# Totoketchup/Adaptive-MultiSpeaker-Separation

Measured on AMD Instinct MI355X. Metric: mixtures/sec training throughput (2-spk, 256-filter adapt+BLSTM-DPCL), higher is better.
Workload: dtype f32 (storage, accumulation and results f32; dense products issued on the 16-bit matrix pipe as fp16x3 / bf16x6 emulation of the f32 product -- `value_native_f32` is the same step on v_mfma_f32_32x32x2_f32)

## Files before the change

adaptive-multispeaker-separation_amd/csrc/common.h:

```cpp
#pragma once
#include <hip/hip_runtime.h>
#include <stdint.h>
#include <stddef.h>
#include "../../include/ams.h"

typedef float f32x4 __attribute__((ext_vector_type(4)));
typedef float f32x16 __attribute__((ext_vector_type(16)));

extern thread_local int g_ams_last_hip_error;

static inline ams_status ams_check_launch() {
    hipError_t e = hipGetLastError();
    if (e != hipSuccess) {
        g_ams_last_hip_error = (int)e;
        return AMS_E_LAUNCH_FAILED;
    }
    return AMS_OK;
}

#define AMS_REQUIRE(cond)            \
    do {                             \
        if (!(cond)) return AMS_E_INVALID_ARG; \
    } while (0)

static inline int ceil_div(long a, long b) { return (int)((a + b - 1) / b); }

namespace ams_detail {
size_t conv_maxpool_ps_bytes(int Bt, int L, int W, int N);
bool conv_maxpool_ps_applies(int Bt, int L, int W, int N);
ams_status conv_maxpool_ps(const float* x, const float* f, float* pmax, int32_t* pidx, int Bt, int L, int W, int N, int pl,
                           const float* amax_x, const float* amax_f, void* img, hipStream_t st);
int dx_splits(int M, int N, int K, size_t ws_bytes, int* kps);
ams_status splitk_reduce(const float* partial, float* C, int M, int N, long ldc, int splits, hipStream_t st);
ams_status conv_fwd_or_dx(const float* x, const float* w, const float* bias, float* y, int M, int N, int T, int F, int lc, int kh, int kw,
                          int rt, int rf, int relu, const float* emask, const float* amax_a, const float* amax_b, float* amax_out,
                          hipStream_t st);
ams_status conv_wgrad(const float* x, const float* dy, float* dw, float* db, float* bsum_ws, int P, int N, int T, int F, int lc, int kh,
                      int kw, int rt, int rf, const float* amax_a, const float* amax_b, void* ws, size_t ws_bytes, hipStream_t st);
size_t conv_wgrad_ws_bytes(int P, int N, int Mrows);
}

__device__ __forceinline__ float wave_sum(float v) {
#pragma unroll
    for (int o = 32; o > 0; o >>= 1) v += __shfl_xor(v, o, 64);
    return v;
}
template <int S>
__device__ __forceinline__ float lane_above(float v) {
    const unsigned b = __builtin_bit_cast(unsigned, v);
    if constexpr (S == 32 || S == 16) {
        unsigned hi = b, lo = 0u;
        if constexpr (S == 32) asm volatile("s_nop 1\n\tv_permlane32_swap_b32 %0, %1\n\ts_nop 1" : "+v"(hi), "+v"(lo));
        else asm volatile("s_nop 1\n\tv_permlane16_swap_b32 %0, %1\n\ts_nop 1" : "+v"(hi), "+v"(lo));
        return __builtin_bit_cast(float, lo);
    }
    else return __builtin_bit_cast(float, __builtin_amdgcn_update_dpp(0u, b, 0x100 | S, 0xf, 0xf, true));
}

__device__ __forceinline__ float wave_sum_lane0(float v) {
    v += lane_above<32>(v);
    v += lane_above<16>(v);
    v += lane_above<8>(v);
    v += lane_above<4>(v);
    v += lane_above<2>(v);
    v += lane_above<1>(v);
// ... 14 lines not shown
```

adaptive-multispeaker-separation_amd/csrc/gemm.hip:

```cpp
#include "common.h"
#include "split.h"
#include <stdlib.h>
#include <atomic>
#include <type_traits>

namespace {

struct LaunchOpt { const float* amax_a = nullptr; const float* amax_b = nullptr; int lds_pad = 0; void* sk_scratch = nullptr; size_t sk_bytes = 0;
                   unsigned* amax_out = nullptr; int force_cfg = -1; };
constexpr size_t AMS_SK_FLAG_BYTES = 8192;
constexpr size_t AMS_SK_SLOT_BYTES = (128 * 256 + 256) * sizeof(float);
std::atomic<int> g_gemm_arith{-1};

struct GemmTuning { int group_m, splits, x6cfg, sk; bool novec, f16x3; };
inline const GemmTuning& tuning() {
    static const GemmTuning t = [] {
        GemmTuning v{0, 0, -1, 1, false, true};
        if (const char* f = getenv("AMS_GEMM_SK")) v.sk = atoi(f);
        if (const char* f = getenv("AMS_GEMM_GROUP_M")) v.group_m = atoi(f);
        if (const char* f = getenv("AMS_GEMM_SPLITS")) v.splits = atoi(f);
        { const char* e = getenv("AMS_GEMM_F16X3"); v.f16x3 = !(e && atoi(e) == 0); }
        v.novec = getenv("AMS_GEMM_NOVEC") != nullptr;
        if (const char* f = getenv("AMS_GEMM_X6CFG")) { const int c = atoi(f); if (c == 0 || c == 3) v.x6cfg = c; }
        return v;
    }();
    return t;
}

#ifndef AMS_GEMM_BK
#define AMS_GEMM_BK 8
#endif
inline bool use_x6() {
    int v = g_gemm_arith.load(std::memory_order_relaxed);
    if (v < 0) {
        const char* f = getenv("AMS_GEMM_X6");
        v = (f && atoi(f) == 0) ? 0 : 1;
        g_gemm_arith.store(v, std::memory_order_relaxed);
    }
    return v != 0;
}
constexpr int BM = 128, BN = 128, BK = AMS_GEMM_BK;
constexpr int X6_BK = 32;
#ifndef AMS_GEMM_X6_US16
#define AMS_GEMM_X6_US16 0.84
#endif
#ifndef AMS_X6_OCC1
#define AMS_X6_OCC1 1
#endif
#ifndef AMS_GEMM_X6_US16_2
#define AMS_GEMM_X6_US16_2 1.35
#endif
constexpr int PAD_T = 2;
constexpr int PAD_V = 4;

enum { A_ROW = 0, A_COL = 1, A_FRAMES = 2, A_FRAMES_T = 3, A_CONV = 4, A_CONV_T = 5 };
// ... 1295 lines not shown
    p.grid = (unsigned)G;
    p.t = wgcu * ((R * nkf + sk_kt) * tk + (R + 1) * 5.0 + 3.0 + 2.0 * contrib) / occ;
    return p;
}

template <int AMODE, int BMODE>
ams_status launch(GemmArgs& g, const LaunchOpt& opt, void* ws, size_t ws_bytes, hipStream_t st, int nbatch = 1,
                  float* bsum_out = nullptr, int bsum_accumulate = 0, float* bsum_ws = nullptr) {
    constexpr bool AKc = (AMODE == A_ROW || AMODE == A_CONV), BKcc = (BMODE == B_COL);
    const int lds_pad = opt.lds_pad < 0 ? 0 : opt.lds_pad;
    const bool capped = lds_pad > 0;
    const bool vec_off = tuning().novec;
    const bool vec = g.a_vec && g.b_vec && !vec_off &&
                     (AMODE == A_FRAMES ? (g.K % 4 == 0 && g.fr_L >= 4) : AMODE == A_FRAMES_T ? (g.M % 4 == 0 && g.fr_L >= 4) :
                      AKc ? (g.K % 4 == 0 && g.K >= 4) : (g.M % 4 == 0 && g.M >= 4)) &&
                     (BKcc ? (g.K % 4 == 0 && g.K >= 4) : (g.N % 4 == 0 && g.N >= 4));
    const bool x6 = vec && use_x6();
    const int cfg = x6 ? ((opt.force_cfg == 0 || opt.force_cfg == 3) && tuning().x6cfg < 0 ? opt.force_cfg : x6_choose_cfg(g.M, g.N)) : 0;
    const bool f16 = x6 && opt.amax_a && opt.amax_b && tuning().f16x3;
    g.amax_a = f16 ? opt.amax_a : nullptr;
    g.amax_b = f16 ? opt.amax_b : nullptr;
    g.amax_out = x6 ? opt.amax_out : nullptr;
    g.c_vec = (g.N % 4 == 0) && (g.ldc % 4 == 0) && (g.c_zs % 4 == 0) && (g.bias_zs % 4 == 0) &&
              (((uintptr_t)g.C | (uintptr_t)ws | (uintptr_t)g.bias) & 15) == 0;
    if (opt.amax_out && !x6) return AMS_E_INVALID_ARG;
    const TilePlan tp = x6 ? x6_plan(cfg) : f32_plan();
    const int tiles = ceil_div(g.M, tp.bm) * ceil_div(g.N, tp.bn);
    g.group_m = choose_group_m(ceil_div(g.M, tp.bm), ceil_div(g.N, tp.bn));
    int splits = 1;
    double t_split = 1e30;
    const bool whole = opt.amax_out || g.relu || g.emask;
    if (ws && !whole) {
        splits = choose_splits(g.M, g.N, g.K, nbatch, tp, &t_split);
        if (tuning().splits > 0) splits = tuning().splits;
        while (splits > 1 && (size_t)nbatch * splits * g.M * g.N * sizeof(float) > ws_bytes) --splits;
    } else choose_splits(g.M, g.N, g.K, nbatch, tp, &t_split, 1);
    int wgcu = 1;
    if (x6 && cfg == 0) { wgcu = capped ? 163840 / (17152 + lds_pad) : 2; if (wgcu < 1) wgcu = 1; if (wgcu > 2) wgcu = 2; }
    SkPlan sk;
    g.sk_rounds = -1; g.sk_flags = nullptr; g.sk_slots = nullptr; g.sk_slot_floats = 0; g.amax_fold = 0;
    if (x6 && !capped && opt.sk_scratch && tuning().sk != 0 && tuning().splits <= 0) {
        sk = sk_plan(tiles * nbatch, g.K, tp, wgcu);
        const size_t slot = (size_t)(tp.bm * tp.bn + tp.bn) * sizeof(float);
        if (sk.rounds >= 0 && (opt.sk_bytes < AMS_SK_FLAG_BYTES + (size_t)sk.grid * slot || (((uintptr_t)opt.sk_scratch) & 15))) sk.rounds = -1;
        if (sk.rounds >= 0 && tuning().sk == 1 && !(sk.t < 0.97 * t_split)) sk.rounds = -1;
        if (sk.rounds == 0 && tuning().sk == 1 && !opt.amax_out) sk.rounds = -1;
        if (sk.rounds >= 0) {
            splits = 1;
            g.sk_rounds = sk.rounds;
            g.sk_flags = (int*)opt.sk_scratch;
            g.sk_slots = (float*)((char*)opt.sk_scratch + AMS_SK_FLAG_BYTES);
            g.sk_slot_floats = (int)(slot / sizeof(float));
        }
    }
    int kps = ceil_div(g.K, splits);
    kps = ceil_div(kps, tp.bk) * tp.bk;
    splits = ceil_div(g.K, kps);
    if (whole && splits > 1) return AMS_E_INVALID_ARG;
    g.splits = splits;
    g.k_per_split = kps;
    g.partial = (float*)ws;
    g.bsum_part = bsum_out ? bsum_ws : nullptr;
    const bool bsum_in_launch = x6 && bsum_out && splits == 1 && (((uintptr_t)bsum_out) & 15) == 0;
    if (sk.rounds >= 0 && bsum_out && !bsum_in_launch) return AMS_E_INVALID_ARG;
    g.bsum_out = bsum_in_launch ? bsum_out : nullptr;
    g.bsum_accumulate = bsum_accumulate;
    g.nbatch = nbatch;
    dim3 grid((unsigned)((long)tiles * splits * nbatch));
// ... 42 lines not shown
    ams_status s = ams_check_launch();
    if (s != AMS_OK) return s;
    if (splits > 1) {
        const long total = (long)g.M * g.N;
        const bool rvec = (g.N % 4 == 0) && (g.ldc % 4 == 0) && (g.c_zs % 4 == 0) && (g.bias_zs % 4 == 0) &&
                          (((uintptr_t)g.C | (uintptr_t)g.partial | (uintptr_t)g.bias) & 15) == 0 && total < (1L << 31);
        if (rvec) {
            int blocks = (int)((total / 4 + 255) / 256);
            if (blocks > 4096) blocks = 4096;
            hipLaunchKernelGGL(splitk_reduce_vec_kernel, dim3(blocks, nbatch), dim3(256), 0, st, g.partial, g.C, g.bias, g.M, g.N, g.ldc,
                               splits, g.accumulate, g.c_zs, g.bias_zs);
        } else {
            int blocks = (int)((total + 255) / 256);
            if (blocks > 2048) blocks = 2048;
            hipLaunchKernelGGL(splitk_reduce_kernel, dim3(blocks, nbatch), dim3(256), 0, st, g.partial, g.C, g.bias, g.M, g.N, g.ldc,
                               splits, g.accumulate, g.c_zs, g.bias_zs);
        }
        s = ams_check_launch();
    }
    if (s == AMS_OK && bsum_out && !bsum_in_launch) {
        if (!vec || BMODE != B_ROW) return AMS_E_INVALID_ARG;
        hipLaunchKernelGGL(bsum_finish_kernel, dim3(ceil_div(g.N, 256)), dim3(256), 0, st, bsum_ws, bsum_out, g.N, splits, bsum_accumulate);
        s = ams_check_launch();
    }
    return s;
}

inline bool aligned16(const void* p) { return ((uintptr_t)p & 15) == 0; }

}

namespace ams_detail {

__attribute__((visibility("hidden"))) int dx_splits(int M, int N, int K, size_t ws_bytes, int* kps) {
    int splits = choose_splits(M, N, K, 1, x6_plan(3));
    if (tuning().splits > 0) splits = tuning().splits;
    while (splits > 1 && (size_t)splits * M * N * sizeof(float) > ws_bytes) --splits;
    int k = ceil_div(ceil_div(K, splits), X6_BK) * X6_BK;
    *kps = k;
    return ceil_div(K, k);
}

__attribute__((visibility("hidden"))) ams_status splitk_reduce(const float* partial, float* C, int M, int N, long ldc, int splits, hipStream_t st) {
    const long total = (long)M * N;
    if (N % 4 || ldc % 4 || (((uintptr_t)C | (uintptr_t)partial) & 15) || total >= (1L << 31)) return AMS_E_INVALID_ARG;
    int blocks = (int)((total / 4 + 255) / 256);
    if (blocks > 4096) blocks = 4096;
    hipLaunchKernelGGL(splitk_reduce_vec_kernel, dim3(blocks, 1), dim3(256), 0, st, partial, C, (const float*)nullptr, M, N, ldc, splits, 0, 0L, 0L);
    return ams_check_launch();
}


__attribute__((visibility("hidden"))) ams_status conv_fwd_or_dx(const float* x, const float* w, const float* bias, float* y, int M, int N,
                                                              int T, int F, int lc, int kh, int kw, int rt, int rf, int relu,
                                                              const float* emask, const float* amax_a, const float* amax_b, float* amax_out,
                                                              hipStream_t st) {
    GemmArgs g{};
    g.A = x; g.B = w; g.C = y; g.bias = bias;
    g.M = M; g.N = N; g.K = kh * kw * (1 << lc); g.lda = 0; g.ldb = N; g.ldc = N;
    g.cv_T = T; g.cv_F = F; g.cv_lc = lc; g.cv_kh = kh; g.cv_kw = kw; g.cv_rt = rt; g.cv_rf = rf;
    g.relu = relu; g.emask = emask;
    g.a_vec = aligned16(x) && lc >= 2;
    g.b_vec = aligned16(w) && (N % 4 == 0);
    LaunchOpt o; o.amax_a = amax_a; o.amax_b = amax_b;
    const bool x6 = use_x6() && g.a_vec && g.b_vec && !tuning().novec && g.K >= 4 && N >= 4;
    if (amax_out && x6) o.amax_out = reinterpret_cast<unsigned*>(amax_out);
    ams_status s = launch<A_CONV, B_ROW>(g, o, nullptr, 0, st);
    if (s == AMS_OK && amax_out && !x6) s = ams_absmax_f32(y, (long)M * N, amax_out, st);
    return s;
}
__attribute__((visibility("hidden"))) ams_status conv_wgrad(const float* x, const float* dy, float* dw, float* db, float* bsum_ws, int P, int N,
                                                          int T, int F, int lc, int kh, int kw, int rt, int rf, const float* amax_a,
                                                          const float* amax_b, void* ws, size_t ws_bytes, hipStream_t st) {
    GemmArgs g{};
    g.A = x; g.B = dy; g.C = dw; g.bias = nullptr;
    g.M = kh * kw * (1 << lc); g.N = N; g.K = P; g.lda = 0; g.ldb = N; g.ldc = N;
    g.cv_T = T; g.cv_F = F; g.cv_lc = lc; g.cv_kh = kh; g.cv_kw = kw; g.cv_rt = rt; g.cv_rf = rf;
    g.a_vec = aligned16(x) && lc >= 2;
    g.b_vec = aligned16(dy) && (N % 4 == 0);
    LaunchOpt o; o.amax_a = amax_a; o.amax_b = amax_b;
    return launch<A_CONV_T, B_ROW>(g, o, ws, ws_bytes, st, 1, db, 0, bsum_ws);
}
size_t conv_wgrad_ws_bytes(int P, int N, int Mrows) { return ams_gemm_workspace_bytes(Mrows, N, P, 1, 0); }

}

extern "C" {

void ams_gemm_set_arith(int mode) { g_gemm_arith.store(mode ? 1 : 0, std::memory_order_relaxed); }
int ams_gemm_get_arith(void) { return use_x6() ? 1 : 0; }

size_t ams_gemm_sk_scratch_bytes(void) {
    const size_t g8 = (size_t)(device_cus() + 7) / 8 * 8;
    const size_t a = g8 * 2 * (128 * 128 + 128) * sizeof(float), b = g8 * AMS_SK_SLOT_BYTES;
    return AMS_SK_FLAG_BYTES + (a > b ? a : b);
}

size_t ams_gemm_workspace_bytes(int M, int N, int K, int nbatch, int lds_pad) {
    if (M <= 0 || N <= 0 || K <= 0 || nbatch <= 0) return 0;
    int splits = choose_splits(M, N, K, nbatch);
    if (tuning().splits > 0) splits = tuning().splits;
    return slab_bytes(M, N, nbatch, splits);
}

ams_status ams_gemm_f32_at_b_colsum(int M, int N, int K, const float* A, long lda, const float* B, long ldb, float* C, long ldc,
                                    int accumulate, float* bsum_out, int bsum_accumulate, float* bsum_ws, const float* amax_a,
                                    const float* amax_b, int lds_pad, void* ws, size_t ws_bytes, void* sk_scratch, size_t sk_bytes,
                                    void* stream) {
    AMS_REQUIRE(M > 0 && N > 0 && K > 0 && A && B && C && bsum_out && bsum_ws);
    GemmArgs g{};
    g.A = A; g.B = B; g.C = C;
    g.M = M; g.N = N; g.K = K; g.lda = lda; g.ldb = ldb; g.ldc = ldc;
    g.accumulate = accumulate;
    g.a_vec = aligned16(A) && (lda % 4 == 0);
    g.b_vec = aligned16(B) && (ldb % 4 == 0);
    AMS_REQUIRE(g.a_vec && g.b_vec && M % 4 == 0 && N % 4 == 0 && aligned16(bsum_ws) && !tuning().novec);
    LaunchOpt o; o.amax_a = amax_a; o.amax_b = amax_b; o.lds_pad = lds_pad; o.sk_scratch = sk_scratch; o.sk_bytes = sk_bytes;
    return launch<A_COL, B_ROW>(g, o, ws, ws_bytes, (hipStream_t)stream, 1, bsum_out, bsum_accumulate, bsum_ws);
}

struct BwGroupPlan { int M[3], N[3], K[3], splits[3], kps[3], tiles_m[3], tiles_n[3]; size_t slab_off[3], bsum_off, bytes; int n_items; };
static bool bw_group_plan(int B, int T, int D, int H, BwGroupPlan& p) {
    if (B <= 0 || T <= 0 || D <= 0 || H <= 0 || D % 4 || H % 4 || (long)B * T < 2 || (long)B * T >= (1L << 31) / (8L * H) ||
        (long)(D + H) * 8 * H >= (1L << 31)) return false;
    const TilePlan tp = x6_plan(3);
    const int Kall = B * T;
    const int M[3] = {D, H, H}, N[3] = {8 * H, 4 * H, 4 * H}, K[3] = {Kall, Kall - 1, Kall - 1};
    int tiles = 0;
    double elems = 0.0;
    for (int r = 0; r < 3; ++r) {
        p.M[r] = M[r]; p.N[r] = N[r]; p.K[r] = K[r];
        p.tiles_m[r] = ceil_div(M[r], tp.bm); p.tiles_n[r] = ceil_div(N[r], tp.bn);
        tiles += p.tiles_m[r] * p.tiles_n[r];
        elems += (double)M[r] * N[r];
// ... 655 lines not shown
```

adaptive-multispeaker-separation_amd/csrc/gemm_ps.hip:

```cpp
#include "common.h"
#include "split.h"
#include <type_traits>

namespace {

typedef __attribute__((address_space(3))) void lds_void;

constexpr int PS_BK = 32, PS_BM = 128, PS_BN = 256, PS_NT = 512;
constexpr int PS_A_BYTES = PS_BM * 128, PS_B_BYTES = PS_BN * 128, PS_STAGE = PS_A_BYTES + PS_B_BYTES;
constexpr int PS_STAGES = 3;
constexpr int PS_BIAS_OFF = PS_STAGES * PS_STAGE;
constexpr int PS_LDS = PS_BIAS_OFF + 2 * 1024;


__device__ __forceinline__ void ps_pack_rows_body(const float* __restrict__ x, long ldx, unsigned char* __restrict__ img,
                                                  unsigned pitch, int R, int K, const float* __restrict__ amax, unsigned block) {
    const int groups = (int)(pitch / 32);
    const long id = (long)block * 256 + threadIdx.x;
    if (id >= (long)R * groups) return;
    const int r = (int)(id / groups), gq = (int)(id - (long)r * groups), k = gq * 8;
    const float s = f16_scale(amax[0]);
    float v[8];
    const float* row = x + (long)r * ldx;
    if (k + 8 <= K && ((((uintptr_t)(row + k)) & 15) == 0)) {
// ... 433 lines not shown
        const bool cok = col < g.N;
        const float4 bv = AF32 ? float4{0.f, 0.f, 0.f, 0.f} : *reinterpret_cast<const float4*>(ps_smem + PS_BIAS_OFF + (wi & 1) * 1024 + (wn * 64 + c4) * 4);
        float* const out = (AF32 && g.splits > 1) ? g.partial + (long)split * g.M * g.N : g.C;
        const long ldo = (AF32 && g.splits > 1) ? (long)g.N : g.ldc;
#pragma unroll
        for (int i = 0; i < 2; ++i) {
#pragma unroll
            for (int j = 0; j < 2; ++j) {
                acc[i][j] = (acc[i][j] + accs[i][j]) * sc_inv;
#pragma unroll
                for (int r = 0; r < 16; ++r) wl[((r & 3) + 8 * (r >> 2) + 4 * lk) * 64 + j * 32 + l31] = acc[i][j][r];
            }
#pragma unroll
            for (int p8 = 0; p8 < 8; ++p8) {
                const int rl = p8 * 4 + rr;
                float4 v = *reinterpret_cast<const float4*>(wl + rl * 64 + c4);
                const int row = em0 + (wm * 2 + i) * 32 + rl;
                if (row < g.M && cok) {
                    if constexpr (!AF32) { v.x += bv.x; v.y += bv.y; v.z += bv.z; v.w += bv.w; }
                    *reinterpret_cast<float4*>(out + (long)row * ldo + col) = v;
                }
            }
        }
        PS_STAMP(2);
        if (more) {
            asm volatile("s_waitcnt lgkmcnt(0)" ::: "memory");
            __builtin_amdgcn_s_barrier();
            if constexpr (AF32) { setup(wi + 1); start_af32(); }
            else if (nk > 1) issue(1, 1);
        }
    }
}

inline int ps_group_m(int tiles_m, int tiles_n) {
    int gm = 8;
    if (gm > tiles_m) gm = tiles_m;
    (void)tiles_n;
    return gm < 1 ? 1 : gm;
}

}

extern "C" {

size_t ams_ps_image_pitch(int K) { return (size_t)((K + 31) / 32) * 128; }
size_t ams_ps_image_bytes(int rows, int K) { return (size_t)rows * ams_ps_image_pitch(K); }

ams_status ams_ps_pack_rows(const float* x, long ldx, void* img, int R, int K, const float* amax, void* stream) {
    AMS_REQUIRE(x && img && amax && R > 0 && K > 0 && ldx >= K && (((uintptr_t)img) & 15) == 0);
    const unsigned pitch = (unsigned)ams_ps_image_pitch(K);
    const long n = (long)R * (pitch / 32);
    hipLaunchKernelGGL(ps_pack_rows_kernel, dim3((unsigned)((n + 255) / 256)), dim3(256), 0, (hipStream_t)stream, x, ldx, (unsigned char*)img, pitch, R, K, amax);
    return ams_check_launch();
}

ams_status ams_ps_pack_cols(const float* w, long ldw, void* img, int K, int N, const float* amax, void* stream) {
    AMS_REQUIRE(w && img && amax && K > 0 && N > 0 && ldw >= N && (((uintptr_t)img) & 15) == 0);
    const unsigned pitch = (unsigned)ams_ps_image_pitch(K);
    hipLaunchKernelGGL(ps_pack_cols_kernel, dim3((unsigned)((N + 63) / 64), (unsigned)(((K + 31) / 32 + PS_PC_KT - 1) / PS_PC_KT)), dim3(256), 0, (hipStream_t)stream, w, ldw,
                       (unsigned char*)img, pitch, K, N, amax);
    return ams_check_launch();
}

ams_status ams_ps_pack_many(const ams_ps_pack_region* regions, int n, int max_workgroups, int lds_pad, void* stream) {
    AMS_REQUIRE(regions && n >= 1 && n <= AMS_PS_PACK_MAX && max_workgroups >= 0 && lds_pad >= 0 && lds_pad <= 150 * 1024);
    PsPackTable tab{};
// ... 12 lines not shown
        tab.r[i] = g;
    }
    tab.blocks = (unsigned)blocks;
    static const bool raised = [] { return hipFuncSetAttribute((const void*)ps_pack_many_kernel, hipFuncAttributeMaxDynamicSharedMemorySize, 150 * 1024) == hipSuccess; }();
    if (!raised) return AMS_E_LAUNCH_FAILED;
    const unsigned grid = (max_workgroups > 0 && (unsigned long)max_workgroups < blocks) ? (unsigned)max_workgroups : (unsigned)blocks;
    hipLaunchKernelGGL(ps_pack_many_kernel, dim3(grid), dim3(256), (size_t)lds_pad, (hipStream_t)stream, tab);
    return ams_check_launch();
}

ams_status ams_gemm_ps(int M, int N, int K, const void* A_img, const void* B_img, float* C, long ldc, const float* bias, const float* amax_a,
                       const float* amax_b, void* stream) {
    AMS_REQUIRE(A_img && B_img && C && amax_a && amax_b && M > 0 && N > 0 && K > 0);
    AMS_REQUIRE(N % 4 == 0 && ldc % 4 == 0 && ldc >= N && ((((uintptr_t)C) | ((uintptr_t)bias) | ((uintptr_t)A_img) | ((uintptr_t)B_img)) & 15) == 0);
    PsArgs g{};
    g.A = (const unsigned char*)A_img; g.B = (const unsigned char*)B_img; g.C = C; g.bias = bias; g.amax_a = amax_a; g.amax_b = amax_b;
    g.M = M; g.N = N; g.K = K; g.ldc = ldc;
    g.pitch_a = g.pitch_b = (unsigned)ams_ps_image_pitch(K);
    AMS_REQUIRE((long)M * g.pitch_a < (1L << 31) && (long)N * g.pitch_b < (1L << 31));
    g.tiles_m = (M + PS_BM - 1) / PS_BM; g.tiles_n = (N + PS_BN - 1) / PS_BN;
    g.group_m = ps_group_m(g.tiles_m, g.tiles_n);
    static const int cus = [] { int dev = 0, n = 0; if (hipGetDevice(&dev) != hipSuccess || hipDeviceGetAttribute(&n, hipDeviceAttributeMultiprocessorCount, dev) != hipSuccess || n <= 0) n = 256; return n; }();
    static const bool raised = [] { return hipFuncSetAttribute((const void*)gemm_ps_kernel<false>, hipFuncAttributeMaxDynamicSharedMemorySize, PS_LDS) == hipSuccess; }();
    if (!raised) return AMS_E_LAUNCH_FAILED;
    const int items = g.tiles_m * g.tiles_n;
    int grid = items < cus ? items : cus;
    if (grid >= 8) grid -= grid % 8;
    hipLaunchKernelGGL(gemm_ps_kernel<false>, dim3((unsigned)grid), dim3(PS_NT), PS_LDS, (hipStream_t)stream, g);
    return ams_check_launch();
}

size_t ams_gemm_ps_a_workspace_bytes(int M, int N, int K) {
    if (M <= 0 || N <= 0 || K <= 0) return 0;
    int kps = 0;
    const int splits = ams_detail::dx_splits(M, N, K, ~(size_t)0, &kps);
    return splits > 1 ? (size_t)splits * M * N * sizeof(float) : 0;
}

ams_status ams_gemm_ps_a_f32(int M, int N, int K, const float* A, long lda, const void* B_img, float* C, long ldc, const float* amax_a,
                             const float* amax_b, void* ws, size_t ws_bytes, void* stream) {
    AMS_REQUIRE(A && B_img && C && amax_a && amax_b && M > 0 && N > 0 && K > 0 && lda >= K);
    AMS_REQUIRE(N % 4 == 0 && ldc % 4 == 0 && ldc >= N && lda % 4 == 0 &&
                ((((uintptr_t)C) | ((uintptr_t)A) | ((uintptr_t)B_img) | ((uintptr_t)ws)) & 15) == 0);
    PsArgs g{};
    g.Af = A; g.lda = lda; g.B = (const unsigned char*)B_img; g.C = C; g.bias = nullptr; g.amax_a = amax_a; g.amax_b = amax_b;
    g.M = M; g.N = N; g.K = K; g.ldc = ldc;
    g.pitch_b = (unsigned)ams_ps_image_pitch(K);
    AMS_REQUIRE((long)M * lda * 4 < (1L << 31) && (long)N * g.pitch_b < (1L << 31));
    g.splits = ams_detail::dx_splits(M, N, K, ws ? ws_bytes : 0, &g.kps);
    g.partial = (float*)ws;
    g.tiles_m = (M + PS_BM - 1) / PS_BM; g.tiles_n = (N + PS_BN - 1) / PS_BN;
    g.group_m = ps_group_m(g.tiles_m, g.tiles_n);
    static const int cus = [] { int dev = 0, n = 0; if (hipGetDevice(&dev) != hipSuccess || hipDeviceGetAttribute(&n, hipDeviceAttributeMultiprocessorCount, dev) != hipSuccess || n <= 0) n = 256; return n; }();
    static const bool raised = [] { return hipFuncSetAttribute((const void*)gemm_ps_kernel<false, true>, hipFuncAttributeMaxDynamicSharedMemorySize, PS_LDS) == hipSuccess; }();
    if (!raised) return AMS_E_LAUNCH_FAILED;
    const int items = g.tiles_m * g.tiles_n * g.splits;
    int grid = items < cus ? items : cus;
    if (grid >= 8) grid -= grid % 8;
    hipLaunchKernelGGL((gemm_ps_kernel<false, true>), dim3((unsigned)grid), dim3(PS_NT), PS_LDS, (hipStream_t)stream, g);
    ams_status r = ams_check_launch();
    if (r == AMS_OK && g.splits > 1) r = ams_detail::splitk_reduce(g.partial, C, M, N, ldc, g.splits, (hipStream_t)stream);
    return r;
}

}

namespace ams_detail {

static inline unsigned conv_lpp(int L, int W) { return (unsigned)((L - 1) / 8 + 4 * ((W + 31) / 32) + 1); }

__attribute__((visibility("hidden"))) size_t conv_maxpool_ps_bytes(int Bt, int L, int W, int N) {
    const size_t a = (size_t)8 * 2 * Bt * conv_lpp(L, W) * 16, b = ams_ps_image_bytes(N, W);
    return (a + 255) / 256 * 256 + (b + 255) / 256 * 256;
}
__attribute__((visibility("hidden"))) bool conv_maxpool_ps_applies(int Bt, int L, int W, int N) {
    return L % PS_BM == 0 && N % 4 == 0 && (size_t)8 * 2 * Bt * conv_lpp(L, W) * 16 < ((size_t)1 << 31) - 64 && ams_ps_image_bytes(N, W) < ((size_t)1 << 31);
}

__attribute__((visibility("hidden"))) ams_status conv_maxpool_ps(const float* x, const float* f, float* pmax, int32_t* pidx, int Bt, int L, int W,
                                                                 int N, int pl, const float* amax_x, const float* amax_f, void* img,
                                                                 hipStream_t st) {
    const unsigned lpp = conv_lpp(L, W);
    const size_t a_bytes = (size_t)8 * 2 * Bt * lpp * 16;
    unsigned char* const ia = (unsigned char*)img;
    unsigned char* const ib = ia + (a_bytes + 255) / 256 * 256;
    const long pieces = (long)8 * Bt * lpp;
    hipLaunchKernelGGL(ps_pack_conv_kernel, dim3((unsigned)((pieces + 255) / 256)), dim3(256), 0, st, x, ia, Bt, L, pl, lpp, amax_x);
    ams_status r = ams_ps_pack_cols(f, N, ib, W, N, amax_f, st);
    if (r != AMS_OK) return r;
    PsArgs g{};
    g.A = ia; g.B = ib; g.C = pmax; g.pidx = pidx; g.bias = nullptr; g.amax_a = amax_x; g.amax_b = amax_f;
    g.M = Bt * L; g.N = N; g.K = W; g.ldc = N;
// ... 16 lines not shown
```

include/ams.h:

```cpp
#ifndef AMS_H
#define AMS_H
#include <stddef.h>
#include <stdint.h>

#ifdef __cplusplus
extern "C" {
#endif

#define AMS_ABI_VERSION 10

typedef int32_t ams_status;
#define AMS_OK 0
#define AMS_E_INVALID_ARG (-1)
#define AMS_E_WORKSPACE_TOO_SMALL (-2)
#define AMS_E_LAUNCH_FAILED (-3)

int ams_last_error(void);
int ams_abi_version(void);

ams_status ams_front_filter_fwd(const float* w, const float* bases, float* f, int W, int N, void* stream);
ams_status ams_front_filter_bwd(const float* w, const float* bases, const float* df, float* dw, float* dbases, int W, int N,
                                void* stream);

size_t ams_front_conv_fwd_workspace_bytes(int Bt, int L, int W, int N, int hop);
// ... 18 lines not shown
                                int P, int hop, int S, void* stream);
ams_status ams_synth_unpool_bwd_vals(const float* dout, const int32_t* pos, const float* f2t, float* dvals, int R, int L, int W, int N,
                                     int T, int S, void* stream);

size_t ams_gemm_workspace_bytes(int M, int N, int K, int nbatch, int lds_pad);
size_t ams_gemm_sk_scratch_bytes(void);
void ams_gemm_set_arith(int mode);
int ams_gemm_get_arith(void);
ams_status ams_gemm_f32(int transA, int transB, int M, int N, int K, const float* A, long lda, const float* B, long ldb, float* C,
                        long ldc, const float* bias, int accumulate, int mask_period, int mask_skip, const float* amax_a,
                        const float* amax_b, int lds_pad, void* ws, size_t ws_bytes, void* sk_scratch, size_t sk_bytes, void* stream);
size_t ams_ps_image_pitch(int K);
size_t ams_ps_image_bytes(int rows, int K);
ams_status ams_ps_pack_rows(const float* x, long ldx, void* img, int R, int K, const float* amax, void* stream);
ams_status ams_ps_pack_cols(const float* w, long ldw, void* img, int K, int N, const float* amax, void* stream);
#define AMS_PS_PACK_MAX 8
#define AMS_PS_PACK_ROWS 0
#define AMS_PS_PACK_COLS 1
typedef struct ams_ps_pack_region {
    const float* src;
    long ld;
    void* img;
    const float* amax;
    int K;
    int rows;
    int kind;
    unsigned pitch;
    unsigned first_block;
} ams_ps_pack_region;
ams_status ams_ps_pack_many(const ams_ps_pack_region* regions, int n, int max_workgroups, int lds_pad, void* stream);
ams_status ams_gemm_ps(int M, int N, int K, const void* A_img, const void* B_img, float* C, long ldc, const float* bias,
                       const float* amax_a, const float* amax_b, void* stream);
size_t ams_gemm_ps_a_workspace_bytes(int M, int N, int K);
ams_status ams_gemm_ps_a_f32(int M, int N, int K, const float* A, long lda, const void* B_img, float* C, long ldc, const float* amax_a,
                             const float* amax_b, void* ws, size_t ws_bytes, void* stream);

ams_status ams_gemm_f32_at_b_colsum(int M, int N, int K, const float* A, long lda, const float* B, long ldb, float* C, long ldc,
                                    int accumulate, float* bsum_out, int bsum_accumulate, float* bsum_ws, const float* amax_a,
                                    const float* amax_b, int lds_pad, void* ws, size_t ws_bytes, void* sk_scratch, size_t sk_bytes,
                                    void* stream);
size_t ams_blstm_bwd_weights_workspace_bytes(int B, int T, int D, int H, int lds_pad);
ams_status ams_blstm_bwd_weights_f32(int B, int T, int D, int H, const float* x, long ldx, const float* h, const float* dz, float* dK,
                                     long ldk, float* db, int accumulate, const float* bound_x, const float* bound_h, const float* bound_dz,
                                     int lds_pad, void* ws, size_t ws_bytes, void* stream);
size_t ams_dilated_conv2d_workspace_bytes(int B, int T, int F, int cin, int cout, int kh, int kw);
ams_status ams_dilated_conv2d_fwd(const float* x, const float* w, const float* bias, float* y, int B, int T, int F, int cin, int cout,
                                  int kh, int kw, int rt, int rf, const float* amax_x, const float* amax_w, float* amax_y, void* ws,
                                  size_t ws_bytes, void* stream);
ams_status ams_dilated_conv2d_bwd_data(const float* dy, const float* w, const float* y_below, float* dx, int B, int T, int F, int cin,
                                       int cout, int kh, int kw, int rt, int rf, const float* amax_dy, const float* amax_w,
                                       float* amax_dx, void* ws, size_t ws_bytes, void* stream);
ams_status ams_dilated_conv2d_bwd_filter(const float* x, const float* dy, float* dw, float* db, int B, int T, int F, int cin,
                                         int cout, int kh, int kw, int rt, int rf, const float* amax_x, const float* amax_dy, void* ws,
                                         size_t ws_bytes, void* stream);
ams_status ams_dilated_conv2d_relu_bwd(const float* dy, const float* y, float* dx, long n, float* amax_dx, void* stream);
ams_status ams_gemm_f32_batched(int transA, int transB, int M, int N, int K, const float* A, long lda, long a_zs, const float* B,
                                long ldb, long b_zs, float* C, long ldc, long c_zs, int nbatch, int accumulate, int mask_period,
                                int mask_skip, const float* amax_a, const float* amax_b, int lds_pad, void* ws, size_t ws_bytes,
                                void* sk_scratch, size_t sk_bytes, void* stream);
ams_status ams_range_share(const float* x, long rows, long cols, long ld, const float* bound, float* out3, void* stream);
ams_status ams_absmax_f32(const float* x, long n, float* out, void* stream);

ams_status ams_make_masks(const float* rep_non_mix, float* Y, int32_t* argmax, int B, int S, long TF, float a, float b,
                          int take_abs, void* stream);

size_t ams_blstm_pack_floats(int H, int backward);
// ... 156 lines not shown
```

Baseline: 24500.

## Add 128x320 wide-tile f16x3 dx GEMM kernel chosen by a cost model

Adds a new pre-split f16x3 GEMM kernel with a 320-column tile: five MFMA blocks per wave, a three-stage B pipeline and direct-to-LDS buffer loads. A planner (dx_plan) compares modeled time for the 256 and 320 tiles and picks the tile and split-K count, and the generic GEMM path and workspace sizing now use it. The aim is more reuse of each A tile and fewer tiles or partial slabs for wide-N data-gradient GEMMs. The cost is higher LDS and register use, one workgroup per CU, and a 320 estimate that is just the 256 per-tile cost scaled by 1.25.

```diff
diff --git a/adaptive-multispeaker-separation_amd/csrc/common.h b/adaptive-multispeaker-separation_amd/csrc/common.h
--- a/adaptive-multispeaker-separation_amd/csrc/common.h
+++ b/adaptive-multispeaker-separation_amd/csrc/common.h
@@ -30,7 +30,8 @@
 bool conv_maxpool_ps_applies(int Bt, int L, int W, int N);
 ams_status conv_maxpool_ps(const float* x, const float* f, float* pmax, int32_t* pidx, int Bt, int L, int W, int N, int pl,
                            const float* amax_x, const float* amax_f, void* img, hipStream_t st);
-int dx_splits(int M, int N, int K, size_t ws_bytes, int* kps);
+struct DxPlan { int tile_n, splits, kps; };
+DxPlan dx_plan(int M, int N, int K, size_t ws_bytes);
 ams_status splitk_reduce(const float* partial, float* C, int M, int N, long ldc, int splits, hipStream_t st);
 ams_status conv_fwd_or_dx(const float* x, const float* w, const float* bias, float* y, int M, int N, int T, int F, int lc, int kh, int kw,
                           int rt, int rf, int relu, const float* emask, const float* amax_a, const float* amax_b, float* amax_out,
diff --git a/adaptive-multispeaker-separation_amd/csrc/gemm.hip b/adaptive-multispeaker-separation_amd/csrc/gemm.hip
--- a/adaptive-multispeaker-separation_amd/csrc/gemm.hip
+++ b/adaptive-multispeaker-separation_amd/csrc/gemm.hip
@@ -12,15 +12,16 @@
 constexpr size_t AMS_SK_SLOT_BYTES = (128 * 256 + 256) * sizeof(float);
 std::atomic<int> g_gemm_arith{-1};
 
-struct GemmTuning { int group_m, splits, x6cfg, sk; bool novec, f16x3; };
+struct GemmTuning { int group_m, splits, x6cfg, sk; bool novec, f16x3; int dx_tile; };
 inline const GemmTuning& tuning() {
     static const GemmTuning t = [] {
-        GemmTuning v{0, 0, -1, 1, false, true};
+        GemmTuning v{0, 0, -1, 1, false, true, 0};
         if (const char* f = getenv("AMS_GEMM_SK")) v.sk = atoi(f);
         if (const char* f = getenv("AMS_GEMM_GROUP_M")) v.group_m = atoi(f);
         if (const char* f = getenv("AMS_GEMM_SPLITS")) v.splits = atoi(f);
         { const char* e = getenv("AMS_GEMM_F16X3"); v.f16x3 = !(e && atoi(e) == 0); }
         v.novec = getenv("AMS_GEMM_NOVEC") != nullptr;
+        if (const char* f = getenv("AMS_GEMM_DX_TILE")) { const int c = atoi(f); if (c == 256 || c == 320) v.dx_tile = c; }
         if (const char* f = getenv("AMS_GEMM_X6CFG")) { const int c = atoi(f); if (c == 0 || c == 3) v.x6cfg = c; }
         return v;
     }();
@@ -1382,8 +1383,11 @@
     const bool whole = opt.amax_out || g.relu || g.emask;
     if (ws && !whole) {
         splits = choose_splits(g.M, g.N, g.K, nbatch, tp, &t_split);
-        if (tuning().splits > 0) splits = tuning().splits;
-        while (splits > 1 && (size_t)nbatch * splits * g.M * g.N * sizeof(float) > ws_bytes) --splits;
+        if (AMODE == A_ROW && BKcc && f16 && cfg == 3 && !capped && nbatch == 1) splits = ams_detail::dx_plan(g.M, g.N, g.K, ws_bytes).splits;
+        else {
+            if (tuning().splits > 0) splits = tuning().splits;
+            while (splits > 1 && (size_t)nbatch * splits * g.M * g.N * sizeof(float) > ws_bytes) --splits;
+        }
     } else choose_splits(g.M, g.N, g.K, nbatch, tp, &t_split, 1);
     int wgcu = 1;
     if (x6 && cfg == 0) { wgcu = capped ? 163840 / (17152 + lds_pad) : 2; if (wgcu < 1) wgcu = 1; if (wgcu > 2) wgcu = 2; }
@@ -1492,13 +1496,21 @@
 
 namespace ams_detail {
 
-__attribute__((visibility("hidden"))) int dx_splits(int M, int N, int K, size_t ws_bytes, int* kps) {
-    int splits = choose_splits(M, N, K, 1, x6_plan(3));
+#ifndef AMS_GEMM_PS320_US16
+#define AMS_GEMM_PS320_US16 (AMS_GEMM_X6_US16_2 * 1.25)
+#endif
+__attribute__((visibility("hidden"))) DxPlan dx_plan(int M, int N, int K, size_t ws_bytes) {
+    double t256 = 1e30, t320 = 1e30;
+    int tile = 256, splits = choose_splits(M, N, K, 1, x6_plan(3), &t256);
+    if (tuning().dx_tile != 256) {
+        const TilePlan p320 = {128, 320, X6_BK, AMS_GEMM_PS320_US16, true};
+        const int s320 = choose_splits(M, N, K, 1, p320, &t320);
+        if ((tuning().dx_tile == 320 || t320 < t256) && slab_bytes(M, N, 1, s320) <= ws_bytes) { tile = 320; splits = s320; }
+    }
     if (tuning().splits > 0) splits = tuning().splits;
     while (splits > 1 && (size_t)splits * M * N * sizeof(float) > ws_bytes) --splits;
-    int k = ceil_div(ceil_div(K, splits), X6_BK) * X6_BK;
-    *kps = k;
-    return ceil_div(K, k);
+    const int k = ceil_div(ceil_div(K, splits), X6_BK) * X6_BK;
+    return {tile, ceil_div(K, k), k};
 }
 
 __attribute__((visibility("hidden"))) ams_status splitk_reduce(const float* partial, float* C, int M, int N, long ldc, int splits, hipStream_t st) {
@@ -1560,6 +1572,10 @@
     if (M <= 0 || N <= 0 || K <= 0 || nbatch <= 0) return 0;
     int splits = choose_splits(M, N, K, nbatch);
     if (tuning().splits > 0) splits = tuning().splits;
+    if (nbatch == 1 && use_x6() && x6_choose_cfg(M, N) == 3) {
+        const int s = ams_detail::dx_plan(M, N, K, ~(size_t)0).splits;
+        if (s > splits) splits = s;
+    }
     return slab_bytes(M, N, nbatch, splits);
 }
 
diff --git a/adaptive-multispeaker-separation_amd/csrc/gemm_ps.hip b/adaptive-multispeaker-separation_amd/csrc/gemm_ps.hip
--- a/adaptive-multispeaker-separation_amd/csrc/gemm_ps.hip
+++ b/adaptive-multispeaker-separation_amd/csrc/gemm_ps.hip
@@ -489,6 +489,217 @@
     }
 }
 
+constexpr int PW_BN = 320, PW_NB = 5;
+constexpr int PW_A_STAGE = PS_BM * 128, PW_B_STAGE = PW_BN * 128;
+constexpr int PW_B_OFF = 2 * PW_A_STAGE, PW_LDS = PW_B_OFF + 3 * PW_B_STAGE;
+static_assert(PW_LDS <= 160 * 1024 && 8 * 4096 <= 3 * PW_B_STAGE, "stages and epilogue patches fit the CU's LDS");
+
+__global__ __launch_bounds__(PS_NT, 1) void gemm_ps_a320_kernel(const PsArgs g) {
+    extern __shared__ __attribute__((aligned(1024))) unsigned char ps_smem[];
+    const int tid = threadIdx.x, lane = tid & 63;
+    const int wave = __builtin_amdgcn_readfirstlane(tid >> 6);
+    const int wm = wave >> 1, wn = wave & 1;
+    const int l31 = lane & 31, lk = lane >> 5;
+    int nk = 0;
+    const int n_items = g.tiles_m * g.tiles_n * g.splits, G = (int)gridDim.x;
+    const int n_work = (n_items - (int)blockIdx.x + G - 1) / G;
+    if (n_work <= 0) return;
+    __builtin_amdgcn_s_setprio(2);
+
+    auto rsrc = [](const unsigned char* p, long bytes) {
+        const unsigned long long a = (unsigned long long)(uintptr_t)p;
+        i32x4_t r = {(int)(unsigned)a, (int)(unsigned)((a >> 32) & 0xffffu), (int)bytes, 0x00020000};
+        r.x = __builtin_amdgcn_readfirstlane(r.x); r.y = __builtin_amdgcn_readfirstlane(r.y);
+        r.z = __builtin_amdgcn_readfirstlane(r.z); r.w = __builtin_amdgcn_readfirstlane(r.w);
+        return r;
+    };
+    const i32x4_t rsA = rsrc(reinterpret_cast<const unsigned char*>(g.Af), (long)g.M * g.lda * 4), rsB = rsrc(g.B, (long)g.N * g.pitch_b);
+
+    const int drow = lane >> 3, dslot = lane & 7;
+    unsigned voffB[PW_NB];
+#pragma unroll
+    for (int q = 0; q < PW_NB; ++q) {
+        const int row = (PW_NB * wave + q) * 8 + drow;
+        voffB[q] = (unsigned)row * g.pitch_b + (unsigned)(dslot ^ ((row >> 1) & 7)) * 16u;
+    }
+
+    const int ff = (l31 >> 1) & 7;
+    unsigned fx[2][2];
+#pragma unroll
+    for (int ks = 0; ks < 2; ++ks)
+#pragma unroll
+        for (int p = 0; p < 2; ++p) fx[ks][p] = (unsigned)(l31 * 128 + (((lk + 2 * ks + 4 * p) ^ ff) * 16));
+
+    const float sc_inv = (1.0f / f16_scale(g.amax_a[0])) * (1.0f / f16_scale(g.amax_b[0]));
+    const float sc_a = f16_scale(g.amax_a[0]);
+
+    int tile_m, tile_n, m0 = 0, n0 = 0, split = 0, kt0 = 0, kend = g.K;
+    const int ar = tid >> 2, ag = tid & 3, af = (ar >> 1) & 7;
+    unsigned avoff = 0;
+    f32x4 ra0 = {}, ra1 = {};
+    auto setup = [&](int i) {
+        ps_locate<true>(g, (int)blockIdx.x + i * G, tile_m, tile_n, split);
+        const unsigned dn = (unsigned)(tile_n * PW_BN - n0) * g.pitch_b;
+        m0 = tile_m * PS_BM; n0 = tile_n * PW_BN;
+        kt0 = split * (g.kps / PS_BK);
+        kend = min(g.K, (split + 1) * g.kps);
+        nk = (kend - kt0 * PS_BK + PS_BK - 1) / PS_BK;
+        int t = tid;
+        asm volatile("" : "+v"(t));
+        avoff = (m0 + (t >> 2) < g.M) ? (unsigned)((long)(m0 + (t >> 2)) * g.lda * 4) + (unsigned)(t & 3) * 32u : 0x80000000u;
+#pragma unroll
+        for (int q = 0; q < PW_NB; ++q) voffB[q] += dn;
+    };
+    const unsigned lds0 = (unsigned)(uintptr_t)(lds_void*)ps_smem;
+    auto issue_b = [&](int kt, int stage, int q) {
+        const unsigned ld = lds0 + (unsigned)(PW_B_OFF + stage * PW_B_STAGE + (PW_NB * wave + q) * 1024);
+        const int ko = (kt0 + kt) * 128;
+        unsigned keep;
+        asm volatile("s_mov_b32 %0, m0\n\ts_mov_b32 m0, %1\n\ts_nop 0\n\tbuffer_load_dwordx4 %2, %3, %4 offen lds\n\ts_mov_b32 m0, %0"
+                     : "=&s"(keep) : "s"(ld), "v"(voffB[q]), "s"(rsB), "s"(ko) : "memory");
+    };
+    auto load_a = [&](int kt) {
+        const unsigned vo = avoff + (unsigned)((kt0 + kt) * 128);
+        asm volatile("s_nop 4\n\tbuffer_load_dwordx4 %0, %2, %3, 0 offen\n\tbuffer_load_dwordx4 %1, %2, %3, 0 offen offset:16"
+                     : "=&v"(ra0), "=&v"(ra1) : "v"(vo), "s"(rsA) : "memory");
+    };
+    auto cut_a = [&](int kt, int stage) {
+        float v[8] = {ra0[0], ra0[1], ra0[2], ra0[3], ra1[0], ra1[1], ra1[2], ra1[3]};
+        const int kb = (kt0 + kt) * PS_BK;
+        if (kb + PS_BK > kend) {
+#pragma unroll
+            for (int j = 0; j < 8; ++j) v[j] = (kb + ag * 8 + j < kend) ? v[j] : 0.f;
+        }
+        uint4 hi, lo;
+        split2h(v[0] * sc_a, v[1] * sc_a, hi.x, lo.x);
+        split2h(v[2] * sc_a, v[3] * sc_a, hi.y, lo.y);
+        split2h(v[4] * sc_a, v[5] * sc_a, hi.z, lo.z);
+        split2h(v[6] * sc_a, v[7] * sc_a, hi.w, lo.w);
+        unsigned char* const p = ps_smem + stage * PW_A_STAGE + ar * 128;
+        *reinterpret_cast<uint4*>(p + ((ag ^ af) * 16)) = hi;
+        *reinterpret_cast<uint4*>(p + (((4 + ag) ^ af) * 16)) = lo;
+    };
+
+    f32x16 acc[PW_NB], accs[PW_NB];
+    auto group = [&](f32x16 (&c)[PW_NB], const f16x8_t& a, const f16x8_t (&b)[PW_NB]) {
+#pragma unroll
+        for (int j = 0; j < PW_NB; ++j) c[j] = __builtin_amdgcn_mfma_f32_32x32x16_f16(a, b[j], c[j], 0, 0, 0);
+#if AMS_PS_SLEEP
+        __builtin_amdgcn_s_sleep(AMS_PS_SLEEP);
+#endif
+    };
+    auto mfma_tile = [&](int sa, int sb, auto PRE, int kt2, int sb2, auto CUT, int sa_c) {
+        constexpr bool pre = decltype(PRE)::value, cut = decltype(CUT)::value;
+        const unsigned char* const pa = ps_smem + sa * PW_A_STAGE + wm * 4096;
+        const unsigned char* const pb = ps_smem + PW_B_OFF + sb * PW_B_STAGE + wn * (PW_NB * 4096);
+        auto rd_a = [&](int ks, int p) { return *reinterpret_cast<const f16x8_t*>(pa + fx[ks][p]); };
+        auto rd_b = [&](f16x8_t (&b)[PW_NB], int ks, int p) {
+            const unsigned char* const q = pb + fx[ks][p];
+#pragma unroll
+            for (int j = 0; j < PW_NB; ++j) b[j] = *reinterpret_cast<const f16x8_t*>(q + j * 4096);
+        };
+        f16x8_t ah0, al0, ah1, al1, bh0[PW_NB], bl0[PW_NB], bh1[PW_NB], bl1[PW_NB];
+        al0 = rd_a(0, 1);
+        rd_b(bh0, 0, 0);
+        ah0 = rd_a(0, 0);
+        rd_b(bl0, 0, 1);
+        __builtin_amdgcn_sched_barrier(0);
+        group(accs, al0, bh0);
+        __builtin_amdgcn_sched_barrier(0);
+        if constexpr (cut) cut_a(kt2 - 1, sa_c);
+        if constexpr (pre) load_a(kt2);
+        __builtin_amdgcn_sched_barrier(0);
+        group(acc, ah0, bh0);
+        __builtin_amdgcn_sched_barrier(0);
+        al1 = rd_a(1, 1);
+        rd_b(bh1, 1, 0);
+        if constexpr (pre) issue_b(kt2, sb2, 0);
+        __builtin_amdgcn_sched_barrier(0);
+        group(accs, ah0, bl0);
+        __builtin_amdgcn_sched_barrier(0);
+        ah1 = rd_a(1, 0);
+        rd_b(bl1, 1, 1);
+        if constexpr (pre) issue_b(kt2, sb2, 1);
+        __builtin_amdgcn_sched_barrier(0);
+        group(accs, al1, bh1);
+        __builtin_amdgcn_sched_barrier(0);
+        if constexpr (pre) issue_b(kt2, sb2, 2);
+        __builtin_amdgcn_sched_barrier(0);
+        group(acc, ah1, bh1);
+        __builtin_amdgcn_sched_barrier(0);
+        if constexpr (pre) { issue_b(kt2, sb2, 3); issue_b(kt2, sb2, 4); }
+        __builtin_amdgcn_sched_barrier(0);
+        group(accs, ah1, bl1);
+    };
+
+    auto start = [&]() {
+        load_a(0);
+        asm volatile("s_waitcnt vmcnt(0)" : "+v"(ra0), "+v"(ra1) :: "memory");
+        cut_a(0, 0);
+#pragma unroll
+        for (int q = 0; q < PW_NB; ++q) issue_b(0, 0, q);
+        if (nk > 1) {
+            load_a(1);
+#pragma unroll
+            for (int q = 0; q < PW_NB; ++q) issue_b(1, 1, q);
+        }
+    };
+    setup(0);
+    start();
+    for (int wi = 0; wi < n_work; ++wi) {
+        PS_STAMP(0);
+#pragma unroll
+        for (int j = 0; j < PW_NB; ++j)
+#pragma unroll
+            for (int r = 0; r < 16; ++r) { acc[j][r] = 0.f; accs[j][r] = 0.f; }
+        int sa = 0, sb = 0;
+        for (int kt = 0; kt < nk - 2; ++kt) {
+            asm volatile("s_waitcnt vmcnt(5) lgkmcnt(0)" : "+v"(ra0), "+v"(ra1) :: "memory");
+            __builtin_amdgcn_s_barrier();
+            mfma_tile(sa, sb, std::true_type{}, kt + 2, sb == 0 ? 2 : sb - 1, std::true_type{}, sa ^ 1);
+            sa ^= 1; sb = sb == 2 ? 0 : sb + 1;
+        }
+        if (nk >= 2) {
+            asm volatile("s_waitcnt vmcnt(5) lgkmcnt(0)" : "+v"(ra0), "+v"(ra1) :: "memory");
+            __builtin_amdgcn_s_barrier();
+            mfma_tile(sa, sb, std::false_type{}, nk, 0, std::true_type{}, sa ^ 1);
+            sa ^= 1; sb = sb == 2 ? 0 : sb + 1;
+        }
+        asm volatile("s_waitcnt vmcnt(0) lgkmcnt(0)" ::: "memory");
+        __builtin_amdgcn_s_barrier();
+        mfma_tile(sa, sb, std::false_type{}, 0, 0, std::false_type{}, 0);
+        PS_STAMP(1);
+        const bool more = wi + 1 < n_work;
+        asm volatile("s_waitcnt lgkmcnt(0)" ::: "memory");
+        __builtin_amdgcn_s_barrier();
+        float* const wl = reinterpret_cast<float*>(ps_smem + PW_B_OFF) + wave * 1024;
+        const int rr = lane >> 3, c4 = (lane & 7) * 4;
+        float* const out = g.splits > 1 ? g.partial + (long)split * g.M * g.N : g.C;
+        const long ldo = g.splits > 1 ? (long)g.N : g.ldc;
+#pragma unroll
+        for (int j = 0; j < PW_NB; ++j) {
+            acc[j] = (acc[j] + accs[j]) * sc_inv;
+#pragma unroll
+            for (int r = 0; r < 16; ++r) wl[((r & 3) + 8 * (r >> 2) + 4 * lk) * 32 + l31] = acc[j][r];
+            const int col = n0 + (wn * PW_NB + j) * 32 + c4;
+#pragma unroll
+            for (int p4 = 0; p4 < 4; ++p4) {
+                const int rl = p4 * 8 + rr;
+                const float4 v = *reinterpret_cast<const float4*>(wl + rl * 32 + c4);
+                const int row = m0 + wm * 32 + rl;
+                if (row < g.M && col < g.N) *reinterpret_cast<float4*>(out + (long)row * ldo + col) = v;
+            }
+        }
+        PS_STAMP(2);
+        if (more) {
+            asm volatile("s_waitcnt lgkmcnt(0)" ::: "memory");
+            __builtin_amdgcn_s_barrier();
+            setup(wi + 1);
+            start();
+        }
+    }
+}
+
 inline int ps_group_m(int tiles_m, int tiles_n) {
     int gm = 8;
     if (gm > tiles_m) gm = tiles_m;
@@ -567,9 +778,15 @@
 
 size_t ams_gemm_ps_a_workspace_bytes(int M, int N, int K) {
     if (M <= 0 || N <= 0 || K <= 0) return 0;
-    int kps = 0;
-    const int splits = ams_detail::dx_splits(M, N, K, ~(size_t)0, &kps);
+    const int splits = ams_detail::dx_plan(M, N, K, ~(size_t)0).splits;
     return splits > 1 ? (size_t)splits * M * N * sizeof(float) : 0;
+}
+
+ams_status ams_gemm_ps_a_plan(int M, int N, int K, size_t ws_bytes, int* tile_n, int* splits, int* kps) {
+    AMS_REQUIRE(M > 0 && N > 0 && K > 0 && tile_n && splits && kps);
+    const ams_detail::DxPlan p = ams_detail::dx_plan(M, N, K, ws_bytes);
+    *tile_n = p.tile_n; *splits = p.splits; *kps = p.kps;
+    return AMS_OK;
 }
 
 ams_status ams_gemm_ps_a_f32(int M, int N, int K, const float* A, long lda, const void* B_img, float* C, long ldc, const float* amax_a,
@@ -582,17 +799,24 @@
     g.M = M; g.N = N; g.K = K; g.ldc = ldc;
     g.pitch_b = (unsigned)ams_ps_image_pitch(K);
     AMS_REQUIRE((long)M * lda * 4 < (1L << 31) && (long)N * g.pitch_b < (1L << 31));
-    g.splits = ams_detail::dx_splits(M, N, K, ws ? ws_bytes : 0, &g.kps);
+    const ams_detail::DxPlan plan = ams_detail::dx_plan(M, N, K, ws ? ws_bytes : 0);
+    const bool wide = plan.tile_n == PW_BN;
+    AMS_REQUIRE(!wide || (long)(N + PW_BN) * g.pitch_b < (1L << 32));
+    g.splits = plan.splits; g.kps = plan.kps;
     g.partial = (float*)ws;
-    g.tiles_m = (M + PS_BM - 1) / PS_BM; g.tiles_n = (N + PS_BN - 1) / PS_BN;
+    g.tiles_m = (M + PS_BM - 1) / PS_BM; g.tiles_n = (N + plan.tile_n - 1) / plan.tile_n;
     g.group_m = ps_group_m(g.tiles_m, g.tiles_n);
     static const int cus = [] { int dev = 0, n = 0; if (hipGetDevice(&dev) != hipSuccess || hipDeviceGetAttribute(&n, hipDeviceAttributeMultiprocessorCount, dev) != hipSuccess || n <= 0) n = 256; return n; }();
-    static const bool raised = [] { return hipFuncSetAttribute((const void*)gemm_ps_kernel<false, true>, hipFuncAttributeMaxDynamicSharedMemorySize, PS_LDS) == hipSuccess; }();
+    static const bool raised = [] {
+        return hipFuncSetAttribute((const void*)gemm_ps_kernel<false, true>, hipFuncAttributeMaxDynamicSharedMemorySize, PS_LDS) == hipSuccess &&
+               hipFuncSetAttribute((const void*)gemm_ps_a320_kernel, hipFuncAttributeMaxDynamicSharedMemorySize, PW_LDS) == hipSuccess;
+    }();
     if (!raised) return AMS_E_LAUNCH_FAILED;
     const int items = g.tiles_m * g.tiles_n * g.splits;
     int grid = items < cus ? items : cus;
     if (grid >= 8) grid -= grid % 8;
-    hipLaunchKernelGGL((gemm_ps_kernel<false, true>), dim3((unsigned)grid), dim3(PS_NT), PS_LDS, (hipStream_t)stream, g);
+    if (wide) hipLaunchKernelGGL(gemm_ps_a320_kernel, dim3((unsigned)grid), dim3(PS_NT), PW_LDS, (hipStream_t)stream, g);
+    else hipLaunchKernelGGL((gemm_ps_kernel<false, true>), dim3((unsigned)grid), dim3(PS_NT), PS_LDS, (hipStream_t)stream, g);
     ams_status r = ams_check_launch();
     if (r == AMS_OK && g.splits > 1) r = ams_detail::splitk_reduce(g.partial, C, M, N, ldc, g.splits, (hipStream_t)stream);
     return r;
diff --git a/include/ams.h b/include/ams.h
--- a/include/ams.h
+++ b/include/ams.h
@@ -74,6 +74,7 @@
 ams_status ams_gemm_ps(int M, int N, int K, const void* A_img, const void* B_img, float* C, long ldc, const float* bias,
                        const float* amax_a, const float* amax_b, void* stream);
 size_t ams_gemm_ps_a_workspace_bytes(int M, int N, int K);
+ams_status ams_gemm_ps_a_plan(int M, int N, int K, size_t ws_bytes, int* tile_n, int* splits, int* kps);
 ams_status ams_gemm_ps_a_f32(int M, int N, int K, const float* A, long lda, const void* B_img, float* C, long ldc, const float* amax_a,
                              const float* amax_b, void* ws, size_t ws_bytes, void* stream);
 
```

Result: faster. 24920, median of 6 (+1.7%).
